# bencebecsy/pta_replicator

Hardware: AMD Instinct MI355X
Metric: realizations/sec, 68 psr x 5000 TOAs GWB+RN+WN (higher is better)
Workload: dtype f64; 1 GPU; BASELINE.json config 3: the 68 pulsars of ng15_dict.json x 5000 synthetic TOAs - HD GWB (gw_log10_A of the dict) + per-pulsar power-law RN (dict values, 30 components) + per-backend EFAC / t2EQUAD / ECORR (dict values), on-chip Philox draws, 1024 realisations per step per GPU; n_toa_total=340000, Nf=3000, npts=600, parallelism=replica-shard x1

## Files before the change

### pta_replicator_amd/csrc/pta_engine_kernels.hip

```cpp
#include "pta_common.h"
#include "pta_rng.h"
#include "pta_mfma.h"

__global__ void k_engine_rn_coef(uint64_t seed, uint64_t r0, int R, int P, int K, const double *__restrict__ amp,
                                 double *__restrict__ coef, int fast) {
  pta_rng_stage_tables();
  __syncthreads();
  int idx = blockIdx.x * blockDim.x + threadIdx.x;
  int hp = K / 2;
  int total = R * P * hp;
  if (idx >= total) return;
  int p = idx % hp, ra = idx / hp;
  int a = ra % P, r = ra / P;
  double z0, z1;
  pta_normal_pair(seed, r0 + (uint64_t)r, pta_stream_id(PTA_STREAM_RN, (uint32_t)a), (uint32_t)p, z0, z1, fast);
  int64_t o = (int64_t)ra * K + 2 * p;
  coef[o] = amp[(int64_t)a * K + 2 * p] * z0;
  coef[o + 1] = amp[(int64_t)a * K + 2 * p + 1] * z1;
}

extern "C" int pta_engine_rn_coef(uint64_t seed, uint64_t r0, int R, int P, int K, const double *amp, double *coef, int rng_fast,
                                  void *stream) {
  PTA_REQUIRE(amp && coef, PTA_E_ARG, "pta_engine_rn_coef: NULL argument");
  PTA_REQUIRE(R > 0 && P > 0 && K > 0 && (K % 2) == 0, PTA_E_ARG, "pta_engine_rn_coef: R=%d P=%d K=%d (K must be even)", R, P, K);
  int64_t total = (int64_t)R * P * (K / 2);
  PTA_REQUIRE(total < (1LL << 31), PTA_E_ARG, "pta_engine_rn_coef: problem too large");
  hipLaunchKernelGGL(k_engine_rn_coef, dim3(pta_cdiv(total, 256)), dim3(256), 0, pta_stream(stream), seed, r0, R, P, K, amp, coef, rng_fast ? 1 : 0);
  PTA_LAUNCH_CHECK();
  return PTA_OK;
}

#define ENG_RB 8

template <int MINW>
__global__ __launch_bounds__(PTA_ENGINE_TILE, MINW) void k_engine_synth(pta_engine_plan pl, uint64_t seed, uint64_t r0, int R,
                                                                  double *__restrict__ out, int64_t ld_out, int fast) {
  __shared__ double zec[ENG_RB][2 * PTA_ENGINE_EPMAX];
  pta_rng_stage_tables();
  __syncthreads();
  const int tile = blockIdx.y;
  const int rb = blockIdx.x * ENG_RB;
  const int a = pl.tile_psr[tile];
  const int start = pl.tile_start[tile];
  const int count = pl.tile_count[tile];
  const int t = threadIdx.x;
  const int P = pl.n_psr;
  const bool has_ec = pl.ecorr_toa != nullptr;
  const int epn = has_ec ? pl.tile_epn[tile] : 0;
  const int ep0 = has_ec ? pl.tile_ep0[tile] : 0;
  if (epn > 0) {
    const uint32_t strm = pta_stream_id(PTA_STREAM_ECORR, (uint32_t)a);
    for (int idx = t; idx < epn * ENG_RB; idx += PTA_ENGINE_TILE) {
      int q = idx / epn, p = idx - q * epn;
      double z0, z1;
      pta_normal_pair(seed, r0 + (uint64_t)(rb + q), strm, (uint32_t)(ep0 + p), z0, z1, fast);
      zec[q][2 * p] = z0;
      zec[q][2 * p + 1] = z1;
    }
    __syncthreads();
  }
  if (t >= count) return;
  const int i = start + t;
  double v[ENG_RB];
#pragma unroll
  for (int q = 0; q < ENG_RB; ++q) v[q] = 0.0;

  if (pl.rn_k > 0) {
    const int K = pl.rn_k;
    const double *__restrict__ Fcol = pl.Ft + i;
    const double *__restrict__ cf = pl.rn_coef + ((int64_t)rb * P + a) * K;
    const int64_t rstride = (int64_t)P * K;
    for (int c = 0; c < K; ++c) {
      double fv = Fcol[(int64_t)c * pl.ldf];
#pragma unroll
      for (int q = 0; q < ENG_RB; ++q) {
        int qq = (rb + q < R) ? q : 0;
        v[q] = fma(fv, cf[qq * rstride + c], v[q]);
      }
    }
  }
  if (pl.gw_npts > 0) {
    const int j = pl.gw_jlo[i];
    const double wgt = pl.gw_w[i];
    const double *__restrict__ gbase = pl.gw_G + ((int64_t)rb * P + a) * pl.gw_npts;
    const int64_t rstride = (int64_t)P * pl.gw_npts;
#pragma unroll
    for (int q = 0; q < ENG_RB; ++q) {
      int qq = (rb + q < R) ? q : 0;
      const double *g = gbase + qq * rstride;
      v[q] = v[q] + ((g[j + 1] - g[j]) * wgt + g[j]);
    }
  }
  if (pl.wn_a) {
    const double wa = pl.wn_a[i], wb = pl.wn_b[i];
    const uint32_t strm = pta_stream_id(PTA_STREAM_WN, (uint32_t)a);
    const uint32_t pair = (uint32_t)pl.idx_in_psr[i];
#pragma unroll
    for (int q = 0; q < ENG_RB; ++q) {
      double z1, z2;
      pta_normal_pair(seed, r0 + (uint64_t)(rb + q), strm, pair, z1, z2, fast);
      v[q] = v[q] + (wa * z1 + wb * z2);
    }
  }
  if (has_ec) {
    const double ec = pl.ecorr_toa[i];
    const int e = pl.epoch_of[i];
    if (epn > 0) {
      const int o = e - 2 * ep0;
#pragma unroll
      for (int q = 0; q < ENG_RB; ++q) v[q] = v[q] + ec * zec[q][o];
    } else if (ec != 0.0) {
      const uint32_t strm = pta_stream_id(PTA_STREAM_ECORR, (uint32_t)a);
#pragma unroll
      for (int q = 0; q < ENG_RB; ++q) v[q] = v[q] + ec * pta_normal_single(seed, r0 + (uint64_t)(rb + q), strm, (uint32_t)e, fast);
    }
  }
  const double det = pl.det ? pl.det[i] : 0.0;
#pragma unroll
  for (int q = 0; q < ENG_RB; ++q)
    if (rb + q < R) out[(int64_t)(rb + q) * ld_out + i] = v[q] + det;
}

typedef double pta_f64x2_a8 __attribute__((ext_vector_type(2), aligned(8)));
#define ENG_MR 16
#define ENG_ZPITCH (2 * PTA_ENGINE_EPMAX + 8)

struct pta_synth_ops {
  pta_f64x2_a8 y[4];
  double wgt, wa, wb, ec, det;
  uint32_t pair;
  int e, i;
};
template <bool FAST, bool SINGLE, bool RNIDX, int PF, int WPC, bool ALL>
__global__ __launch_bounds__(PTA_ENGINE_TILE, WPC) void k_engine_synth_mfma(pta_engine_plan pl, uint64_t seed, uint64_t r0, int R,
                                                                           double *__restrict__ out, int64_t ld_out, int xcd_aware) {
  constexpr int fast = FAST ? 1 : 0;
  __shared__ double zec[ENG_MR][ENG_ZPITCH];
  const int nrg = (R + ENG_MR - 1) / ENG_MR;
  const int64_t total = (int64_t)nrg * pl.n_tiles, chunk = (total + 7) >> 3;
  const int64_t item = xcd_aware ? (int64_t)(blockIdx.x & 7) * chunk + (blockIdx.x >> 3) : (int64_t)blockIdx.x;
  if (item >= total) return;
  pta_rng_stage_tables();
  __syncthreads();
  const int t = threadIdx.x, l = t & 63, wv = t >> 6;
  const int P = pl.n_psr;
  const bool has_ec = ALL || pl.ecorr_toa != nullptr;
  constexpr bool wn_single = SINGLE;
  const int col = l & 15, quad = l >> 4;
  const int tbase = wv * 64 + col;
  const int tile = (int)(item / nrg);
  const int rb = (int)(item - (int64_t)tile * nrg) * ENG_MR;
  const int a = pl.tile_psr[tile];
  const int start = pl.tile_start[tile];
  const int count = pl.tile_count[tile];
  const int epn = has_ec ? pl.tile_epn[tile] : 0;
  const int ep0 = has_ec ? pl.tile_ep0[tile] : 0;
  auto stage = [&]() {
    if (epn > 0) {
      const uint32_t strm = pta_stream_id(PTA_STREAM_ECORR, (uint32_t)a);
      for (int idx = t; idx < epn * ENG_MR; idx += PTA_ENGINE_TILE) {
        int q = idx / epn, p = idx - q * epn;
        double z0, z1;
        pta_normal_pair(seed, r0 + (uint64_t)(rb + q), strm, (uint32_t)(ep0 + p), z0, z1, fast);
        zec[q][2 * p] = z0;
        zec[q][2 * p + 1] = z1;
      }
      __syncthreads();
    }
  };
  if (PF == 0) stage();
  int rq[4];
#pragma unroll
  for (int g = 0; g < 4; ++g) rq[g] = min(quad + 4 * g, R - 1 - rb);
  int jl4[4];
#pragma unroll
  for (int j = 0; j < 4; ++j) jl4[j] = pl.gw_npts > 0 ? pl.gw_jlo[start + min(tbase + 16 * j, count - 1)] : 0;
  pta_f64x4 acc[4];
#pragma unroll
  for (int j = 0; j < 4; ++j) acc[j] = pta_f64x4{0.0, 0.0, 0.0, 0.0};
  const bool has_gw = ALL || pl.gw_npts > 0, has_wn = ALL || pl.wn_a != nullptr || wn_single;
  auto ldgw = [&](int j, pta_synth_ops &o) {
    const int i = start + min(tbase + 16 * j, count - 1);
    o.wgt = has_gw ? pl.gw_w[i] : 0.0;
    if (has_gw) {
#pragma unroll
      for (int g = 0; g < 4; ++g)
        o.y[g] = *reinterpret_cast<const pta_f64x2_a8 *>(pl.gw_G + ((int64_t)(rb + rq[g]) * P + a) * pl.gw_npts + jl4[j]);
    }
  };
  auto ldtoa = [&](int j, pta_synth_ops &o) {
    const int i = start + min(tbase + 16 * j, count - 1);
    o.i = i;
    o.wa = has_wn ? (wn_single ? pl.wn_c[i] : pl.wn_a[i]) : 0.0;
    o.wb = (has_wn && !wn_single) ? pl.wn_b[i] : 0.0;
    o.pair = (uint32_t)pl.idx_in_psr[i];
    o.ec = has_ec ? pl.ecorr_toa[i] : 0.0;
    o.e = has_ec ? pl.epoch_of[i] : 0;
    o.det = pl.det ? pl.det[i] : 0.0;
  };
  pta_synth_ops cur;
  auto mid = [&]() {
    if (PF & 4) ldgw(0, cur);
    if (PF & 1) ldtoa(0, cur);
    stage();
  };
  if (PF != 0 && !(PF & 2)) mid();
  if (pl.rn_k > 0) {
    const int K = pl.rn_k;
    const int ra = min(rb + col, R - 1);
    const double *__restrict__ cf = pl.rn_coef + ((int64_t)ra * P + a) * K;
    const double *__restrict__ Fb = pl.Ft + start;
    int tcl[4];
#pragma unroll
    for (int j = 0; j < 4; ++j) tcl[j] = min(tbase + 16 * j, count - 1);
    auto ld = [&](int k0, double &av, double (&bv)[4]) {
      const int k = k0 + quad, kc = min(k, K - 1);
      const double a_ld = cf[kc];
      av = (k < K) ? a_ld : 0.0;
      const double *__restrict__ Fk = Fb + (int64_t)kc * pl.ldf;
#pragma unroll
      for (int j = 0; j < 4; ++j) bv[j] = Fk[tcl[j]];
    };
    auto mm = [&](double av, const double (&bv)[4]) {
#pragma unroll
      for (int j = 0; j < 4; ++j) acc[j] = pta_mfma_f64(av, bv[j], acc[j]);
    };
    auto run = [&](auto &&ldx) {
      double a0, a1, a2, b0[4], b1[4], b2[4];
      ldx(0, a0, b0);
      ldx(4, a1, b1);
      if (PF & 2) mid();
      for (int k0 = 0; k0 < K; k0 += 12) {
        ldx(k0 + 8, a2, b2);
        mm(a0, b0);
        ldx(k0 + 12, a0, b0);
        mm(a1, b1);
        ldx(k0 + 16, a1, b1);
        mm(a2, b2);
      }
    };
    if (RNIDX) {
      const int klast = (K - 1) & ~3;
      const char *__restrict__ Fbytes = reinterpret_cast<const char *>(Fb);
      const char *__restrict__ cbytes = reinterpret_cast<const char *>(pl.rn_coef);
      const uint32_t ldfb = (uint32_t)pl.ldf * 8u;
      uint32_t offF[4];
#pragma unroll
      for (int j = 0; j < 4; ++j) offF[j] = (uint32_t)quad * ldfb + (uint32_t)tcl[j] * 8u;
      const uint32_t offC = (uint32_t)(((int64_t)ra * P + a) * K + quad) * 8u;
      const int kq = K - quad;
      auto ldu = [&](int k0, auto rowF, auto rowC, double &av, double (&bv)[4]) {
        const double a_ld = *reinterpret_cast<const double *>(cbytes + (uint32_t)(offC + rowC));
        av = (k0 < kq) ? a_ld : 0.0;
#pragma unroll
        for (int j = 0; j < 4; ++j) bv[j] = *reinterpret_cast<const double *>(Fbytes + (uint32_t)(offF[j] + rowF));
      };
      if ((K & 3) == 0) {
        run([&](int k0, double &av, double (&bv)[4]) {
          const uint32_t kg = (uint32_t)min(k0, klast);
          ldu(k0, kg * ldfb, kg * 8u, av, bv);
        });
      } else {
        const uint32_t dq = (uint32_t)(quad - min(quad, K - 1 - klast));
        run([&](int k0, double &av, double (&bv)[4]) {
          const uint32_t kg = (uint32_t)min(k0, klast);
          const uint32_t back = k0 >= klast ? dq : 0u;
          ldu(k0, kg * ldfb - back * ldfb, kg * 8u - back * 8u, av, bv);
        });
      }
    } else {
      run(ld);
    }
  } else if (PF & 2) {
    mid();
  }
  const uint32_t strm_wn = pta_stream_id(PTA_STREAM_WN, (uint32_t)a);
  const uint32_t strm_ec = pta_stream_id(PTA_STREAM_ECORR, (uint32_t)a);
  const bool wn_share = wn_single && count == PTA_ENGINE_TILE;
  double zs[4] = {0.0, 0.0, 0.0, 0.0};
  double pend[4] = {0.0, 0.0, 0.0, 0.0};
  int pend_i = 0;
#pragma unroll
  for (int j = 0; j < 4; ++j) {
    pta_synth_ops nxt;
    if (PF & 4) {
      if (!(PF & 1)) ldtoa(j, cur);
      if (j < 3) {
        ldgw(j + 1, nxt);
        if (PF & 1) ldtoa(j + 1, nxt);
      }
    }
    double wgt, wa, wb, ec, det;
    uint32_t pair;
    int e, i;
    pta_f64x2_a8 y[4];
    if (PF & 4) {
      wgt = cur.wgt, wa = cur.wa, wb = cur.wb, ec = cur.ec, det = cur.det, pair = cur.pair, e = cur.e, i = cur.i;
#pragma unroll
      for (int g = 0; g < 4; ++g) y[g] = cur.y[g];
    } else {
      i = start + min(tbase + 16 * j, count - 1);
      wgt = has_gw ? pl.gw_w[i] : 0.0;
      if (has_gw) {
#pragma unroll
        for (int g = 0; g < 4; ++g)
          y[g] = *reinterpret_cast<const pta_f64x2_a8 *>(pl.gw_G + ((int64_t)(rb + rq[g]) * P + a) * pl.gw_npts + jl4[j]);
      }
      wa = has_wn ? (wn_single ? pl.wn_c[i] : pl.wn_a[i]) : 0.0, wb = (has_wn && !wn_single) ? pl.wn_b[i] : 0.0;
      pair = (uint32_t)pl.idx_in_psr[i];
      ec = has_ec ? pl.ecorr_toa[i] : 0.0;
      e = has_ec ? pl.epoch_of[i] : 0;
      det = pl.det ? pl.det[i] : 0.0;
    }
    if (j > 0) {
#pragma unroll
      for (int g = 0; g < 4; ++g) out[(int64_t)(rb + rq[g]) * ld_out + pend_i] = pend[g];
    }
    double v[4];
#pragma unroll
    for (int g = 0; g < 4; ++g) v[g] = acc[j][g];
    if (has_gw) {
#pragma unroll
      for (int g = 0; g < 4; ++g) v[g] = v[g] + ((y[g].y - y[g].x) * wgt + y[g].x);
    }
    if (has_wn && !wn_single) {
#pragma unroll
      for (int g = 0; g < 4; ++g) {
        double z1, z2;
        pta_normal_pair(seed, r0 + (uint64_t)(rb + rq[g]), strm_wn, pair, z1, z2, fast);
        v[g] = v[g] + (wa * z1 + wb * z2);
      }
    } else if (wn_single) {
      const uint32_t pid = pair & ~16u;
      const bool br = (pair & 16u) != 0;
      const bool fresh = (j & 1) == 0 || !wn_share;
      if (fresh) {
#pragma unroll
        for (int g = 0; g < 4; ++g) {
          double z0, z1;
          pta_normal_pair(seed, r0 + (uint64_t)(rb + rq[g]), strm_wn, pid, z0, z1, fast);
          v[g] = v[g] + wa * (br ? z1 : z0);
          zs[g] = br ? z0 : z1;
        }
      } else {
#pragma unroll
        for (int g = 0; g < 4; ++g) v[g] = v[g] + wa * zs[g];
      }
    }
    if (has_ec) {
      if (epn > 0) {
        const int o = e - 2 * ep0;
#pragma unroll
        for (int g = 0; g < 4; ++g) v[g] = v[g] + ec * zec[rq[g]][o];
      }
#ifndef PTA_ISA_TABLE_MAIN_PATH_ONLY
      else if (ec != 0.0) {
#pragma unroll
        for (int g = 0; g < 4; ++g) v[g] = v[g] + ec * pta_normal_single(seed, r0 + (uint64_t)(rb + rq[g]), strm_ec, (uint32_t)e, fast);
      }
#endif
    }
#pragma unroll
    for (int g = 0; g < 4; ++g) pend[g] = v[g] + det;
    pend_i = i;
    if ((PF & 4) && j < 3) {
      cur.wgt = nxt.wgt;
#pragma unroll
      for (int g = 0; g < 4; ++g) cur.y[g] = nxt.y[g];
      if (PF & 1) cur = nxt;
    }
  }
#pragma unroll
  for (int g = 0; g < 4; ++g) out[(int64_t)(rb + rq[g]) * ld_out + pend_i] = pend[g];
}

typedef void (*pta_synth_fn)(pta_engine_plan, uint64_t, uint64_t, int, double *, int64_t, int);
template <bool FAST, bool SINGLE, bool RNIDX, int WPC, bool ALL>
static pta_synth_fn synth_kernel_pf(int pf) {
  if (pf == 0) return k_engine_synth_mfma<FAST, SINGLE, RNIDX, 0, WPC, ALL>;
  if (pf == 2) return k_engine_synth_mfma<FAST, SINGLE, RNIDX, 2, WPC, ALL>;
  if constexpr (WPC == 3) {
    if (pf == 4) return k_engine_synth_mfma<FAST, SINGLE, RNIDX, 4, WPC, ALL>;
    if (pf == 6) return k_engine_synth_mfma<FAST, SINGLE, RNIDX, 6, WPC, ALL>;
    if constexpr (!SINGLE) {
      if (pf == 5) return k_engine_synth_mfma<FAST, SINGLE, RNIDX, 5, WPC, ALL>;
      if (pf == 7) return k_engine_synth_mfma<FAST, SINGLE, RNIDX, 7, WPC, ALL>;
    }
  }
  return nullptr;
}
template <bool RNIDX, bool ALL>
static pta_synth_fn synth_kernel(int rng_fast, bool single, int pf, bool w3) {
  if (single) return rng_fast ? synth_kernel_pf<true, true, RNIDX, 3, ALL>(pf) : synth_kernel_pf<false, true, RNIDX, 3, ALL>(pf);
  if (w3) return rng_fast ? synth_kernel_pf<true, false, RNIDX, 3, ALL>(pf) : synth_kernel_pf<false, false, RNIDX, 3, ALL>(pf);
  return rng_fast ? synth_kernel_pf<true, false, RNIDX, 4, ALL>(pf) : synth_kernel_pf<false, false, RNIDX, 4, ALL>(pf);
}
#define PTA_SYNTH_DEFAULT_PF 0
#define PTA_SYNTH_DEFAULT_WPC 4

extern "C" int pta_engine_synth(const pta_engine_plan *plan_host, uint64_t seed, uint64_t r0, int R, double *out, int64_t ld_out,
                                void *stream) {
  PTA_REQUIRE(plan_host && out, PTA_E_ARG, "pta_engine_synth: NULL argument");
  const pta_engine_plan &p = *plan_host;
  PTA_REQUIRE(p.n_toa > 0 && p.n_psr > 0 && R > 0 && ld_out >= p.n_toa, PTA_E_ARG, "pta_engine_synth: n_toa=%d n_psr=%d R=%d", p.n_toa,
              p.n_psr, R);
  PTA_REQUIRE(p.n_tiles > 0 && p.tile_psr && p.tile_start && p.tile_count && p.tile_ep0 && p.tile_epn && p.idx_in_psr, PTA_E_ARG,
              "pta_engine_synth: tile table / idx_in_psr missing");
  PTA_REQUIRE(p.rn_k == 0 || (p.Ft && p.rn_coef && p.ldf >= p.n_toa), PTA_E_ARG, "pta_engine_synth: red-noise inputs missing");
  PTA_REQUIRE(p.gw_npts == 0 || (p.gw_G && p.gw_jlo && p.gw_w && p.gw_npts >= 2), PTA_E_ARG,
              "pta_engine_synth: GWB inputs missing");
  PTA_REQUIRE(!p.wn_a || p.wn_b, PTA_E_ARG, "pta_engine_synth: wn_b missing");
  PTA_REQUIRE(!p.wn_c || !p.wn_a, PTA_E_ARG, "pta_engine_synth: wn_c (single-deviate white noise) replaces wn_a / wn_b - pass one or the other");
  PTA_REQUIRE(!p.ecorr_toa || p.epoch_of, PTA_E_ARG, "pta_engine_synth: epoch_of missing");
  const int variant = p.synth_variant;
  const int rng_fast = p.rng_fast ? 1 : 0;
  const bool pipe = variant >= 16 && variant <= 79;
  PTA_REQUIRE(!pipe || (((variant - 16) & 7) != 1 && ((variant - 16) & 7) != 3), PTA_E_ARG,
              "pta_engine_synth: synth_variant %d - per-TOA operands ahead (bit 0) exist with the GWB operands ahead (bit 2) only", variant);
  if (variant == 0 || variant == 1 || variant == 2 || pipe || (variant >= 100 && variant <= 164)) {
    const int xcd = variant == 1 ? 0 : 1;
    const unsigned pad = variant >= 100 ? (unsigned)(variant - 100) * 1024u : 0u;
    const int64_t total = (int64_t)pta_cdiv(R, ENG_MR) * p.n_tiles, nwg = ((total + 7) >> 3) << 3;
    PTA_REQUIRE(nwg < (1LL << 31), PTA_E_ARG, "pta_engine_synth: %lld workgroups exceed one launch", (long long)nwg);
    const bool noidx = variant == 2 || (pipe && ((variant - 16) & 16));
    const bool rnidx = !noidx && p.rn_k > 0 && p.ldf < (1LL << 28) && ((int64_t)p.rn_k * p.ldf + PTA_ENGINE_TILE) * 8 < (1LL << 32) &&
                       (int64_t)R * p.n_psr * p.rn_k * 8 < (1LL << 32);
    const int pf = pipe ? (variant - 16) & 7 : variant == 2 ? 0 : PTA_SYNTH_DEFAULT_PF;
    const bool w3 = p.wn_c || (pipe ? ((variant - 16) & 8) != 0 : variant == 2 ? false : PTA_SYNTH_DEFAULT_WPC == 3);
    const bool all = !(pipe && ((variant - 16) & 32)) && variant != 2 && p.gw_npts > 0 && (p.wn_a || p.wn_c) && p.ecorr_toa;
    pta_synth_fn kern = all ? (rnidx ? synth_kernel<true, true>(rng_fast, p.wn_c != nullptr, pf, w3) : synth_kernel<false, true>(rng_fast, p.wn_c != nullptr, pf, w3))
                            : (rnidx ? synth_kernel<true, false>(rng_fast, p.wn_c != nullptr, pf, w3) : synth_kernel<false, false>(rng_fast, p.wn_c != nullptr, pf, w3));
    PTA_REQUIRE(kern, PTA_E_ARG, "pta_engine_synth: synth_variant %d - no kernel with pipelining %d at %d workgroups per CU%s (scratch)", variant, pf,
                w3 ? 3 : 4, p.wn_c ? ", single-deviate white noise" : "");
    hipLaunchKernelGGL(kern, dim3((unsigned)nwg), dim3(PTA_ENGINE_TILE), pad, pta_stream(stream), p, seed, r0, R, out, ld_out, xcd);
    PTA_LAUNCH_CHECK();
    return PTA_OK;
  }
  PTA_REQUIRE(!p.wn_c, PTA_E_ARG, "pta_engine_synth: the single-deviate white noise exists in the MFMA kernel only");
  PTA_REQUIRE(p.n_tiles <= 65535, PTA_E_ARG, "pta_engine_synth: %d tiles exceed the 2-D launch of the all-VALU kernel", p.n_tiles);
  dim3 g(pta_cdiv(R, ENG_RB), p.n_tiles), b(PTA_ENGINE_TILE);
  if (variant >= 8)
    hipLaunchKernelGGL(k_engine_synth<8>, g, b, 0, pta_stream(stream), p, seed, r0, R, out, ld_out, rng_fast);
  else if (variant >= 6)
    hipLaunchKernelGGL(k_engine_synth<6>, g, b, 0, pta_stream(stream), p, seed, r0, R, out, ld_out, rng_fast);
  else
    hipLaunchKernelGGL(k_engine_synth<4>, g, b, 0, pta_stream(stream), p, seed, r0, R, out, ld_out, rng_fast);
  PTA_LAUNCH_CHECK();
  return PTA_OK;
}

extern "C" int pta_gwb_czt(uint64_t seed, uint64_t r0, const double *w, int64_t ldw, int R, int P, int Nf, int npts, int i0,
                           const double *pre, const double *FB, const double *tw, const double *post, double *G0, int64_t ldg,
                           int variant, int rng_fast, void *stream);
extern "C" int pta_gwb_idft_rng(uint64_t seed, uint64_t r0, int R, int P, int Nf, const double *Tsym, const double *rot, int npts,
                                double *G0, int64_t ldg, int variant, int rng_fast, void *stream);
extern "C" int pta_gwb_mix(const double *Mchol, int P, const double *G0, int R, int npts, int64_t ldg, double *G, int variant,
                           void *stream);

static int engine_generate(const char *fn, const pta_engine_plan *plan_host, const pta_engine_tables *tables_host,
                           const pta_engine_hyper *hyper, uint64_t seed, uint64_t r0, int R, double *out, int64_t ld_out, void *stream) {
  PTA_REQUIRE(plan_host && tables_host && out, PTA_E_ARG, "%s: NULL argument", fn);
  const pta_engine_hyper fixed{};
  const pta_engine_hyper &h = hyper ? *hyper : fixed;
  pta_engine_plan p = *plan_host;
  const pta_engine_tables &tb = *tables_host;
  int rc;
  if (p.rn_k > 0) {
    PTA_REQUIRE(tb.rn_amp && tb.ws_coef, PTA_E_ARG, "%s: red-noise amplitudes / workspace missing", fn);
    if (h.rn_log10_A) {
      PTA_REQUIRE(h.rn_gamma && h.rn_f && h.rn_tspan, PTA_E_ARG, "%s: rn_gamma / rn_f / rn_tspan missing", fn);
      rc = pta_engine_rn_coef_hyper(seed, r0, R, p.n_psr, p.rn_k, h.rn_f, h.rn_tspan, h.rn_log10_A, h.rn_gamma, tb.rn_amp, tb.ws_coef,
                                    p.rng_fast, stream);
    } else {
      rc = pta_engine_rn_coef(seed, r0, R, p.n_psr, p.rn_k, tb.rn_amp, tb.ws_coef, p.rng_fast, stream);
    }
    if (rc != PTA_OK) return rc;
    p.rn_coef = tb.ws_coef;
  }
  if (p.gw_npts > 0) {
    PTA_REQUIRE(tb.Mchol && tb.ws_G0 && tb.ws_G, PTA_E_ARG, "%s: GWB factor / workspace missing", fn);
    const double *scale = h.gw_scale;
    if (!scale && h.gw_log10_A) {
      PTA_REQUIRE(h.gw_gamma && h.gw_f && h.gw_hcf0 && h.ws_scale, PTA_E_ARG, "%s: gw_gamma / gw_f / gw_hcf0 / ws_scale missing", fn);
      rc = pta_gwb_spectrum_scale(h.gw_f, h.gw_hcf0, tb.gw_nf, R, h.gw_log10_A, h.gw_gamma, h.gw_turnover, h.gw_f0, h.gw_beta,
                                  h.gw_power, h.ws_scale, h.ld_gw_scale, stream);
      if (rc != PTA_OK) return rc;
      scale = h.ws_scale;
    }
    if (tb.use_czt) {
      PTA_REQUIRE(tb.czt_pre && tb.czt_FB && tb.czt_tw && tb.czt_post, PTA_E_ARG, "%s: chirp-z tables missing", fn);
      rc = scale ? pta_gwb_czt_scaled(seed, r0, nullptr, 0, R, p.n_psr, tb.gw_nf, p.gw_npts, tb.gw_i0, tb.czt_pre, tb.czt_FB, tb.czt_tw,
                                      tb.czt_post, tb.ws_G0, p.gw_npts, tb.czt_variant, p.rng_fast, scale, h.ld_gw_scale, stream)
                 : pta_gwb_czt(seed, r0, nullptr, 0, R, p.n_psr, tb.gw_nf, p.gw_npts, tb.gw_i0, tb.czt_pre, tb.czt_FB, tb.czt_tw,
                               tb.czt_post, tb.ws_G0, p.gw_npts, tb.czt_variant, p.rng_fast, stream);
    } else {
      PTA_REQUIRE(tb.Tsym && tb.rot, PTA_E_ARG, "%s: DFT-GEMM tables missing", fn);
      rc = scale ? pta_gwb_idft_rng_scaled(seed, r0, R, p.n_psr, tb.gw_nf, tb.Tsym, tb.rot, p.gw_npts, tb.ws_G0, p.gw_npts, tb.idft_variant,
                                           p.rng_fast, scale, h.ld_gw_scale, stream)
                 : pta_gwb_idft_rng(seed, r0, R, p.n_psr, tb.gw_nf, tb.Tsym, tb.rot, p.gw_npts, tb.ws_G0, p.gw_npts, tb.idft_variant,
                                    p.rng_fast, stream);
    }
    if (rc != PTA_OK) return rc;
    rc = pta_gwb_mix(tb.Mchol, p.n_psr, tb.ws_G0, R, p.gw_npts, p.gw_npts, tb.ws_G, tb.mix_variant, stream);
    if (rc != PTA_OK) return rc;
    p.gw_G = tb.ws_G;
  }
  return pta_engine_synth(&p, seed, r0, R, out, ld_out, stream);
}

extern "C" int pta_engine_generate(const pta_engine_plan *plan_host, const pta_engine_tables *tables_host, uint64_t seed, uint64_t r0,
                                   int R, double *out, int64_t ld_out, void *stream) {
  return engine_generate("pta_engine_generate", plan_host, tables_host, nullptr, seed, r0, R, out, ld_out, stream);
}

extern "C" int pta_engine_generate_hyper(const pta_engine_plan *plan_host, const pta_engine_tables *tables_host,
                                         const pta_engine_hyper *hyper_host, uint64_t seed, uint64_t r0, int R, double *out,
                                         int64_t ld_out, void *stream) {
  PTA_REQUIRE(hyper_host, PTA_E_ARG, "pta_engine_generate_hyper: NULL argument");
  return engine_generate("pta_engine_generate_hyper", plan_host, tables_host, hyper_host, seed, r0, R, out, ld_out, stream);
}
```

### pta_replicator_amd/csrc/pta_rng.h

```cpp
#pragma once
#include <stdint.h>
#include <math.h>
#include "pta_rng_tables.h"

#ifndef PTA_HD
#if defined(__HIPCC__)
#define PTA_HD __host__ __device__ __forceinline__
#else
#define PTA_HD inline
#endif
#endif

#define PTA_STREAM_GWB 1u
#define PTA_STREAM_RN 2u
#define PTA_STREAM_WN 3u
#define PTA_STREAM_ECORR 4u
#define PTA_STREAM_TD 5u
#define PTA_STREAM_TDGW 6u
#define PTA_STREAM_HYPER 7u
#define PTA_STREAM_CW 8u

PTA_HD uint32_t pta_stream_id(uint32_t kind, uint32_t pulsar) { return (kind << 24) | (pulsar & 0xFFFFFFu); }

struct pta_u32x4 {
  uint32_t x, y, z, w;
};

PTA_HD void pta_mulhilo32(uint32_t a, uint32_t b, uint32_t &hi, uint32_t &lo) {
  uint64_t p = (uint64_t)a * (uint64_t)b;
  hi = (uint32_t)(p >> 32);
  lo = (uint32_t)p;
}

PTA_HD uint32_t pta_xor3(uint32_t a, uint32_t b, uint32_t c) {
#if defined(__HIP_DEVICE_COMPILE__)
  return __builtin_amdgcn_bitop3_b32(a, b, c, 0x96);
#else
  return a ^ b ^ c;
#endif
}

PTA_HD pta_u32x4 pta_philox4x32_10(pta_u32x4 c, uint32_t k0, uint32_t k1) {
#pragma unroll
  for (int r = 0; r < 10; ++r) {
    uint32_t hi0, lo0, hi1, lo1;
    pta_mulhilo32(0xD2511F53u, c.x, hi0, lo0);
    pta_mulhilo32(0xCD9E8D57u, c.z, hi1, lo1);
    pta_u32x4 n;
    n.x = pta_xor3(hi1, c.y, k0);
    n.y = lo1;
    n.z = pta_xor3(hi0, c.w, k1);
    n.w = lo0;
    c = n;
    k0 += 0x9E3779B9u;
    k1 += 0xBB67AE85u;
  }
  return c;
}

PTA_HD pta_u32x4 pta_philox_draw(uint64_t seed, uint64_t realisation, uint32_t stream, uint32_t pair) {
  pta_u32x4 c;
  c.x = pair;
  c.y = stream;
  c.z = (uint32_t)realisation;
  c.w = (uint32_t)(realisation >> 32);
  return pta_philox4x32_10(c, (uint32_t)seed, (uint32_t)(seed >> 32));
}

PTA_HD double pta_bits_to_double(uint64_t b) {
  double d;
  __builtin_memcpy(&d, &b, sizeof(d));
  return d;
}
PTA_HD uint64_t pta_double_to_bits(double d) {
  uint64_t b;
  __builtin_memcpy(&b, &d, sizeof(b));
  return b;
}

PTA_HD void pta_uniform_pair(pta_u32x4 v, double &u1, double &u2) {
  uint64_t a = ((((uint64_t)v.x << 32) | v.y) >> 12) | 0x3FF0000000000000ull;
  uint64_t b = ((((uint64_t)v.z << 32) | v.w) >> 12) | 0x3FF0000000000000ull;
  u1 = 2.0 - pta_bits_to_double(a);
  u2 = pta_bits_to_double(b) - 1.0;
}

PTA_HD double pta_fma_k(double x, double p, double c) {
#if defined(__HIP_DEVICE_COMPILE__)
  double d;
  asm("v_fma_f64 %0, %1, %2, %3" : "=v"(d) : "v"(x), "v"(p), "s"(c));
  return d;
#else
  return fma(x, p, c);
#endif
}

PTA_HD double pta_div(double x, double y) {
#if defined(__HIP_DEVICE_COMPILE__)
  double r = __builtin_amdgcn_rcp(y);
  r = fma(fma(-y, r, 1.0), r, r);
  double q = x * r;
  return fma(fma(-y, q, x), r, q);
#else
  return x / y;
#endif
}
PTA_HD double pta_sqrt_pos(double x) {
#if defined(__HIP_DEVICE_COMPILE__)
  x = fmax(x, 1e-300);
  double r = __builtin_amdgcn_rsq(x);
  double g = x * r, h = 0.5 * r;
  double d = fma(-h, g, 0.5);
  g = fma(g, d, g);
  h = fma(h, d, h);
  return fma(fma(-g, g, x), h, g);
#else
  return sqrt(fmax(x, 1e-300));
#endif
}

PTA_HD double pta_neg2log_poly(double u) {
  const double ln2_hi = 6.93147180369123816490e-01, ln2_lo = 1.90821492927058770002e-10;
  const double Lg1 = 6.666666666666735130e-01, Lg2 = 3.999999999940941908e-01, Lg3 = 2.857142874366239149e-01,
               Lg4 = 2.222219843214978396e-01, Lg5 = 1.818357216161805012e-01, Lg6 = 1.531383769920937332e-01,
               Lg7 = 1.479819860511658591e-01;
  uint64_t b = pta_double_to_bits(u);
  int e = (int)(b >> 52) - 1023;
  double m = pta_bits_to_double((b & 0x000FFFFFFFFFFFFFull) | 0x3FF0000000000000ull);
  if (m > 1.4142135623730951) {
    m *= 0.5;
    e += 1;
  }
  double f = m - 1.0;
  double s = pta_div(f, 2.0 + f);
  double z = s * s, w = z * z;
  double t1 = w * pta_fma_k(w, fma(w, Lg6, Lg4), Lg2);
  double t2 = z * pta_fma_k(w, pta_fma_k(w, fma(w, Lg7, Lg5), Lg3), Lg1);
  double R = t2 + t1;
  double hfsq = 0.5 * f * f;
  double dk = (double)e;
  double lnu = dk * ln2_hi - ((hfsq - fma(s, hfsq + R, dk * ln2_lo)) - f);
  return -2.0 * lnu;
}

PTA_HD void pta_sincos_2pi_poly(double u, double &sn, double &cs) {
  const double S1 = -1.66666666666666324348e-01, S2 = 8.33333333332248946124e-03, S3 = -1.98412698298579493134e-04,
               S4 = 2.75573137070700676789e-06, S5 = -2.50507602534068634195e-08, S6 = 1.58969099521155010221e-10;
  const double C1 = 4.16666666666666019037e-02, C2 = -1.38888888888741095749e-03, C3 = 2.48015872894767294178e-05,
               C4 = -2.75573143513906633035e-07, C5 = 2.08757232129817482790e-09, C6 = -1.13596475577881948265e-11;
  double q = rint(4.0 * u);
  double r = u - 0.25 * q;
  double x = 6.283185307179586 * r;
  double z = x * x;
  double ps = pta_fma_k(z, pta_fma_k(z, pta_fma_k(z, pta_fma_k(z, fma(z, S6, S5), S4), S3), S2), S1);
  double s = fma(x * z, ps, x);
  double pc = z * pta_fma_k(z, pta_fma_k(z, pta_fma_k(z, pta_fma_k(z, fma(z, C6, C5), C4), C3), C2), C1);
  double c = 1.0 - (0.5 * z - z * pc);
  int k = (int)q & 3;
  double s1 = (k & 1) ? c : s;
  double c1 = (k & 1) ? s : c;
  sn = (k == 2 || k == 3) ? -s1 : s1;
  cs = (k == 1 || k == 2) ? -c1 : c1;
}


#if defined(__HIP_DEVICE_COMPILE__)
__device__ __forceinline__ double *pta_rng_lds() {
  __shared__ double __attribute__((aligned(16))) tab[PTA_RNG_TAB_DOUBLES];
  return tab;
}
__device__ __forceinline__ void pta_rng_stage_tables() {
  double *t = pta_rng_lds();
  for (int i = threadIdx.x + blockDim.x * (threadIdx.y + blockDim.y * threadIdx.z); i < PTA_RNG_TAB_DOUBLES; i += blockDim.x * blockDim.y * blockDim.z)
    t[i] = pta_rng_tab[i];
}
#define PTA_RNG_TABLE pta_rng_lds()
#else
PTA_HD void pta_rng_stage_tables() {}
#define PTA_RNG_TABLE pta_rng_tab
#endif

PTA_HD double pta_neg2log(double u) {
  const double L2H = 1.38629436073824763298e+00, L2L = 3.81642985854117540004e-10;
  const uint64_t b = pta_double_to_bits(u);
  const uint32_t hi = (uint32_t)(b >> 32);
  const uint32_t j = (hi >> (20 - PTA_RNG_LOG_BITS)) & ((1u << PTA_RNG_LOG_BITS) - 1u);
  const int nk = 1023 - (int)((hi + (((1u << PTA_RNG_LOG_BITS) - PTA_RNG_LOG_CENTRED) << (20 - PTA_RNG_LOG_BITS))) >> 20);
  const uint32_t hi2 = hi + ((uint32_t)nk << 20);
  const double m = pta_bits_to_double(((uint64_t)hi2 << 32) | (b & 0xFFFFFFFFull));
  const double *e = PTA_RNG_TABLE + 2 * j;
  const double c = e[0], T = e[1];
  const double r = fma(m, c, -1.0);
  const double W = pta_fma_k(r, pta_fma_k(r, pta_fma_k(r, pta_fma_k(r, fma(r, -2.85714285714285698425e-01, 3.33333333333333314830e-01),
                                                   -4.00000000000000022204e-01), 0.5), -6.66666666666666629659e-01), 1.0);
  const double t = fma(r * r, W, -2.0 * r);
  const double nkd = (double)nk;
  return fma(nkd, L2H, T + fma(nkd, L2L, t));
}

PTA_HD void pta_sincos_2pi(double u, double &sn, double &cs) {
  const double kd = rint((double)PTA_RNG_SC_N * u);
  const double r = fma(kd, -1.0 / PTA_RNG_SC_N, u);
  const int k = (int)kd & (PTA_RNG_SC_N - 1);
  const double *e = PTA_RNG_TABLE + PTA_RNG_SC_OFF + 2 * k;
  const double sa = e[0], ca = e[1];
  const double x = 6.283185307179586 * r;
  const double z = x * x;
  const double ps = pta_fma_k(z, pta_fma_k(z, pta_fma_k(z, fma(z, 2.75573192239858925110e-06, -1.98412698412698412526e-04), 8.33333333333333321769e-03),
                                       -1.66666666666666657415e-01), 1.0);
  const double cx = pta_fma_k(z, pta_fma_k(z, pta_fma_k(z, fma(z, 2.48015873015873015658e-05, -1.38888888888888894189e-03), 4.16666666666666643537e-02),
                                       -0.5), 1.0);
  const double sx = x * ps;
  sn = fma(sa, cx, ca * sx);
  cs = fma(ca, cx, -(sa * sx));
}

PTA_HD void pta_normal_pair(uint64_t seed, uint64_t realisation, uint32_t stream, uint32_t pair, double &z0, double &z1, int fast = 0) {
  double u1, u2, s, c;
  pta_uniform_pair(pta_philox_draw(seed, realisation, stream, pair), u1, u2);
  if (fast) {
#if defined(__HIP_DEVICE_COMPILE__)
    float rad = __builtin_amdgcn_sqrtf(-1.3862943611198906f * __builtin_amdgcn_logf((float)u1));
    float x = (float)u2;
    z0 = (double)(rad * __builtin_amdgcn_cosf(x));
    z1 = (double)(rad * __builtin_amdgcn_sinf(x));
#else
    float rad = sqrtf(-1.3862943611198906f * log2f((float)u1));
    float x = 6.2831853071795864769f * (float)u2;
    z0 = (double)(rad * cosf(x));
    z1 = (double)(rad * sinf(x));
#endif
    return;
  }
  double rad = pta_sqrt_pos(pta_neg2log(u1));
  pta_sincos_2pi(u2, s, c);
  z0 = rad * c;
  z1 = rad * s;
}

PTA_HD double pta_normal_single(uint64_t seed, uint64_t realisation, uint32_t stream, uint32_t e, int fast = 0) {
  double z0, z1;
  pta_normal_pair(seed, realisation, stream, e >> 1, z0, z1, fast);
  return (e & 1u) ? z1 : z0;
}
```

Baseline: 216,400 realizations/s.

## Split first Philox round into per-realisation and per-pair halves shared via LDS

```diff
diff --git a/pta_replicator_amd/csrc/pta_engine_kernels.hip b/pta_replicator_amd/csrc/pta_engine_kernels.hip
--- a/pta_replicator_amd/csrc/pta_engine_kernels.hip
+++ b/pta_replicator_amd/csrc/pta_engine_kernels.hip
@@ -1,6 +1,7 @@
 #include "pta_common.h"
 #include "pta_rng.h"
 #include "pta_mfma.h"
+#include <type_traits>
 
 __global__ void k_engine_rn_coef(uint64_t seed, uint64_t r0, int R, int P, int K, const double *__restrict__ amp,
                                  double *__restrict__ coef, int fast) {
@@ -131,7 +132,11 @@
   uint32_t pair;
   int e, i;
 };
-template <bool FAST, bool SINGLE, bool RNIDX, int PF, int WPC, bool ALL>
+__device__ __forceinline__ uint4 *pta_synth_rhalf_lds() {
+  __shared__ uint4 tab[2 * ENG_MR];
+  return tab;
+}
+template <bool FAST, bool SINGLE, bool RNIDX, int PF, int WPC, bool ALL, bool SPLIT = false>
 __global__ __launch_bounds__(PTA_ENGINE_TILE, WPC) void k_engine_synth_mfma(pta_engine_plan pl, uint64_t seed, uint64_t r0, int R,
                                                                            double *__restrict__ out, int64_t ld_out, int xcd_aware) {
   constexpr int fast = FAST ? 1 : 0;
@@ -141,22 +146,47 @@
   const int64_t item = xcd_aware ? (int64_t)(blockIdx.x & 7) * chunk + (blockIdx.x >> 3) : (int64_t)blockIdx.x;
   if (item >= total) return;
   pta_rng_stage_tables();
+  const int t = threadIdx.x, l = t & 63, wv = t >> 6;
+  const int tile = (int)(item / nrg);
+  const int rb = (int)(item - (int64_t)tile * nrg) * ENG_MR;
+  const int a = pl.tile_psr[tile];
+  const uint32_t r_hi = (uint32_t)((r0 + (uint64_t)rb) >> 32);
+  const bool split_ok = SPLIT && r_hi == (uint32_t)((r0 + (uint64_t)rb + (ENG_MR - 1)) >> 32);
+  if constexpr (SPLIT) {
+    if (t < 2 * ENG_MR) {
+      const bool is_ec = t >= ENG_MR;
+      const int q = is_ec ? t - ENG_MR : min(t, R - 1 - rb);
+      const pta_philox_half B = pta_philox_real_half((uint32_t)(r0 + (uint64_t)(rb + q)), pta_stream_id(is_ec ? PTA_STREAM_ECORR : PTA_STREAM_WN, (uint32_t)a), seed);
+      pta_synth_rhalf_lds()[t] = make_uint4(B.a, B.b, B.c, 0u);
+    }
+  }
   __syncthreads();
-  const int t = threadIdx.x, l = t & 63, wv = t >> 6;
+  auto body = [&](auto sp_c) {
+  constexpr bool SP = decltype(sp_c)::value;
   const int P = pl.n_psr;
   const bool has_ec = ALL || pl.ecorr_toa != nullptr;
   constexpr bool wn_single = SINGLE;
   const int col = l & 15, quad = l >> 4;
   const int tbase = wv * 64 + col;
-  const int tile = (int)(item / nrg);
-  const int rb = (int)(item - (int64_t)tile * nrg) * ENG_MR;
-  const int a = pl.tile_psr[tile];
   const int start = pl.tile_start[tile];
   const int count = pl.tile_count[tile];
   const int epn = has_ec ? pl.tile_epn[tile] : 0;
   const int ep0 = has_ec ? pl.tile_ep0[tile] : 0;
   auto stage = [&]() {
     if (epn > 0) {
+      if constexpr (SP) {
+        const int q = t >> 4;
+        const uint4 b = pta_synth_rhalf_lds()[ENG_MR + q];
+        const pta_philox_half B = {b.x, b.y, b.z};
+        for (int p = t & 15; p < epn; p += 16) {
+          double z0, z1;
+          pta_normal_pair_split(pta_philox_pair_half((uint32_t)(ep0 + p), r_hi, seed), B, seed, z0, z1, fast);
+          zec[q][2 * p] = z0;
+          zec[q][2 * p + 1] = z1;
+        }
+        __syncthreads();
+        return;
+      }
       const uint32_t strm = pta_stream_id(PTA_STREAM_ECORR, (uint32_t)a);
       for (int idx = t; idx < epn * ENG_MR; idx += PTA_ENGINE_TILE) {
         int q = idx / epn, p = idx - q * epn;
@@ -280,6 +310,11 @@
   double zs[4] = {0.0, 0.0, 0.0, 0.0};
   double pend[4] = {0.0, 0.0, 0.0, 0.0};
   int pend_i = 0;
+  [[maybe_unused]] const uint4 *rhalf = pta_synth_rhalf_lds() + quad;
+  auto draw = [&](pta_philox_half A, int g, double &z0, double &z1) {
+    const uint4 b = rhalf[4 * g];
+    pta_normal_pair_split(A, pta_philox_half{b.x, b.y, b.z}, seed, z0, z1, fast);
+  };
 #pragma unroll
   for (int j = 0; j < 4; ++j) {
     pta_synth_ops nxt;
@@ -324,10 +359,13 @@
       for (int g = 0; g < 4; ++g) v[g] = v[g] + ((y[g].y - y[g].x) * wgt + y[g].x);
     }
     if (has_wn && !wn_single) {
+      pta_philox_half A;
+      if constexpr (SP) A = pta_philox_pair_half(pair, r_hi, seed);
 #pragma unroll
       for (int g = 0; g < 4; ++g) {
         double z1, z2;
-        pta_normal_pair(seed, r0 + (uint64_t)(rb + rq[g]), strm_wn, pair, z1, z2, fast);
+        if constexpr (SP) draw(A, g, z1, z2);
+        else pta_normal_pair(seed, r0 + (uint64_t)(rb + rq[g]), strm_wn, pair, z1, z2, fast);
         v[g] = v[g] + (wa * z1 + wb * z2);
       }
     } else if (wn_single) {
@@ -335,10 +373,13 @@
       const bool br = (pair & 16u) != 0;
       const bool fresh = (j & 1) == 0 || !wn_share;
       if (fresh) {
+        pta_philox_half A;
+        if constexpr (SP) A = pta_philox_pair_half(pid, r_hi, seed);
 #pragma unroll
         for (int g = 0; g < 4; ++g) {
           double z0, z1;
-          pta_normal_pair(seed, r0 + (uint64_t)(rb + rq[g]), strm_wn, pid, z0, z1, fast);
+          if constexpr (SP) draw(A, g, z0, z1);
+          else pta_normal_pair(seed, r0 + (uint64_t)(rb + rq[g]), strm_wn, pid, z0, z1, fast);
           v[g] = v[g] + wa * (br ? z1 : z0);
           zs[g] = br ? z0 : z1;
         }
@@ -372,11 +413,23 @@
   }
 #pragma unroll
   for (int g = 0; g < 4; ++g) out[(int64_t)(rb + rq[g]) * ld_out + pend_i] = pend[g];
+  };
+  if constexpr (SPLIT) {
+    if (split_ok) body(std::true_type{});
+    else body(std::false_type{});
+  } else {
+    body(std::false_type{});
+  }
 }
 
 typedef void (*pta_synth_fn)(pta_engine_plan, uint64_t, uint64_t, int, double *, int64_t, int);
 template <bool FAST, bool SINGLE, bool RNIDX, int WPC, bool ALL>
-static pta_synth_fn synth_kernel_pf(int pf) {
+static pta_synth_fn synth_kernel_pf(int pf, bool split) {
+  if constexpr (WPC == 4 || SINGLE) {
+    if (split) return pf == 0 ? k_engine_synth_mfma<FAST, SINGLE, RNIDX, 0, WPC, ALL, true> : nullptr;
+  } else {
+    if (split) return nullptr;
+  }
   if (pf == 0) return k_engine_synth_mfma<FAST, SINGLE, RNIDX, 0, WPC, ALL>;
   if (pf == 2) return k_engine_synth_mfma<FAST, SINGLE, RNIDX, 2, WPC, ALL>;
   if constexpr (WPC == 3) {
@@ -390,10 +443,10 @@
   return nullptr;
 }
 template <bool RNIDX, bool ALL>
-static pta_synth_fn synth_kernel(int rng_fast, bool single, int pf, bool w3) {
-  if (single) return rng_fast ? synth_kernel_pf<true, true, RNIDX, 3, ALL>(pf) : synth_kernel_pf<false, true, RNIDX, 3, ALL>(pf);
-  if (w3) return rng_fast ? synth_kernel_pf<true, false, RNIDX, 3, ALL>(pf) : synth_kernel_pf<false, false, RNIDX, 3, ALL>(pf);
-  return rng_fast ? synth_kernel_pf<true, false, RNIDX, 4, ALL>(pf) : synth_kernel_pf<false, false, RNIDX, 4, ALL>(pf);
+static pta_synth_fn synth_kernel(int rng_fast, bool single, int pf, bool w3, bool split) {
+  if (single) return rng_fast ? synth_kernel_pf<true, true, RNIDX, 3, ALL>(pf, split) : synth_kernel_pf<false, true, RNIDX, 3, ALL>(pf, split);
+  if (w3) return rng_fast ? synth_kernel_pf<true, false, RNIDX, 3, ALL>(pf, split) : synth_kernel_pf<false, false, RNIDX, 3, ALL>(pf, split);
+  return rng_fast ? synth_kernel_pf<true, false, RNIDX, 4, ALL>(pf, split) : synth_kernel_pf<false, false, RNIDX, 4, ALL>(pf, split);
 }
 #define PTA_SYNTH_DEFAULT_PF 0
 #define PTA_SYNTH_DEFAULT_WPC 4
@@ -417,7 +470,7 @@
   const bool pipe = variant >= 16 && variant <= 79;
   PTA_REQUIRE(!pipe || (((variant - 16) & 7) != 1 && ((variant - 16) & 7) != 3), PTA_E_ARG,
               "pta_engine_synth: synth_variant %d - per-TOA operands ahead (bit 0) exist with the GWB operands ahead (bit 2) only", variant);
-  if (variant == 0 || variant == 1 || variant == 2 || pipe || (variant >= 100 && variant <= 164)) {
+  if (variant == 0 || variant == 1 || variant == 2 || variant == 3 || pipe || (variant >= 100 && variant <= 164)) {
     const int xcd = variant == 1 ? 0 : 1;
     const unsigned pad = variant >= 100 ? (unsigned)(variant - 100) * 1024u : 0u;
     const int64_t total = (int64_t)pta_cdiv(R, ENG_MR) * p.n_tiles, nwg = ((total + 7) >> 3) << 3;
@@ -427,9 +480,10 @@
                        (int64_t)R * p.n_psr * p.rn_k * 8 < (1LL << 32);
     const int pf = pipe ? (variant - 16) & 7 : variant == 2 ? 0 : PTA_SYNTH_DEFAULT_PF;
     const bool w3 = p.wn_c || (pipe ? ((variant - 16) & 8) != 0 : variant == 2 ? false : PTA_SYNTH_DEFAULT_WPC == 3);
+    const bool split = variant == 0 || variant == 1 || variant >= 100;
     const bool all = !(pipe && ((variant - 16) & 32)) && variant != 2 && p.gw_npts > 0 && (p.wn_a || p.wn_c) && p.ecorr_toa;
-    pta_synth_fn kern = all ? (rnidx ? synth_kernel<true, true>(rng_fast, p.wn_c != nullptr, pf, w3) : synth_kernel<false, true>(rng_fast, p.wn_c != nullptr, pf, w3))
-                            : (rnidx ? synth_kernel<true, false>(rng_fast, p.wn_c != nullptr, pf, w3) : synth_kernel<false, false>(rng_fast, p.wn_c != nullptr, pf, w3));
+    pta_synth_fn kern = all ? (rnidx ? synth_kernel<true, true>(rng_fast, p.wn_c != nullptr, pf, w3, split) : synth_kernel<false, true>(rng_fast, p.wn_c != nullptr, pf, w3, split))
+                            : (rnidx ? synth_kernel<true, false>(rng_fast, p.wn_c != nullptr, pf, w3, split) : synth_kernel<false, false>(rng_fast, p.wn_c != nullptr, pf, w3, split));
     PTA_REQUIRE(kern, PTA_E_ARG, "pta_engine_synth: synth_variant %d - no kernel with pipelining %d at %d workgroups per CU%s (scratch)", variant, pf,
                 w3 ? 3 : 4, p.wn_c ? ", single-deviate white noise" : "");
     hipLaunchKernelGGL(kern, dim3((unsigned)nwg), dim3(PTA_ENGINE_TILE), pad, pta_stream(stream), p, seed, r0, R, out, ld_out, xcd);
diff --git a/pta_replicator_amd/csrc/pta_rng.h b/pta_replicator_amd/csrc/pta_rng.h
--- a/pta_replicator_amd/csrc/pta_rng.h
+++ b/pta_replicator_amd/csrc/pta_rng.h
@@ -67,6 +67,48 @@
   return pta_philox4x32_10(c, (uint32_t)seed, (uint32_t)(seed >> 32));
 }
 
+struct pta_philox_half {
+  uint32_t a, b, c;
+};
+PTA_HD pta_philox_half pta_philox_pair_half(uint32_t pair, uint32_t realisation_hi, uint64_t seed) {
+  uint32_t hi0, lo0;
+  pta_philox_half h;
+  pta_mulhilo32(0xD2511F53u, pair, hi0, lo0);
+  pta_mulhilo32(0xCD9E8D57u, pta_xor3(hi0, realisation_hi, (uint32_t)(seed >> 32)), h.a, h.b);
+  h.c = lo0;
+  return h;
+}
+PTA_HD pta_philox_half pta_philox_real_half(uint32_t realisation_lo, uint32_t stream, uint64_t seed) {
+  uint32_t hi1;
+  pta_philox_half h;
+  pta_mulhilo32(0xCD9E8D57u, realisation_lo, hi1, h.a);
+  pta_mulhilo32(0xD2511F53u, pta_xor3(hi1, stream, (uint32_t)seed), h.b, h.c);
+  return h;
+}
+PTA_HD pta_u32x4 pta_philox_join(pta_philox_half A, pta_philox_half B, uint64_t seed) {
+  uint32_t k0 = (uint32_t)seed + 0x9E3779B9u, k1 = (uint32_t)(seed >> 32) + 0xBB67AE85u;
+  pta_u32x4 c;
+  c.x = pta_xor3(A.a, B.a, k0);
+  c.y = A.b;
+  c.z = pta_xor3(B.b, A.c, k1);
+  c.w = B.c;
+#pragma unroll
+  for (int r = 2; r < 10; ++r) {
+    k0 += 0x9E3779B9u;
+    k1 += 0xBB67AE85u;
+    uint32_t hi0, lo0, hi1, lo1;
+    pta_mulhilo32(0xD2511F53u, c.x, hi0, lo0);
+    pta_mulhilo32(0xCD9E8D57u, c.z, hi1, lo1);
+    pta_u32x4 n;
+    n.x = pta_xor3(hi1, c.y, k0);
+    n.y = lo1;
+    n.z = pta_xor3(hi0, c.w, k1);
+    n.w = lo0;
+    c = n;
+  }
+  return c;
+}
+
 PTA_HD double pta_bits_to_double(uint64_t b) {
   double d;
   __builtin_memcpy(&d, &b, sizeof(d));
@@ -78,9 +120,16 @@
   return b;
 }
 
+PTA_HD uint64_t pta_mantissa_12(uint32_t x, uint32_t y) {
+#if defined(__HIP_DEVICE_COMPILE__)
+  return ((uint64_t)__builtin_amdgcn_alignbit(0x3FFu, x, 12) << 32) | __builtin_amdgcn_alignbit(x, y, 12);
+#else
+  return ((((uint64_t)x << 32) | y) >> 12) | 0x3FF0000000000000ull;
+#endif
+}
 PTA_HD void pta_uniform_pair(pta_u32x4 v, double &u1, double &u2) {
-  uint64_t a = ((((uint64_t)v.x << 32) | v.y) >> 12) | 0x3FF0000000000000ull;
-  uint64_t b = ((((uint64_t)v.z << 32) | v.w) >> 12) | 0x3FF0000000000000ull;
+  uint64_t a = pta_mantissa_12(v.x, v.y);
+  uint64_t b = pta_mantissa_12(v.z, v.w);
   u1 = 2.0 - pta_bits_to_double(a);
   u2 = pta_bits_to_double(b) - 1.0;
 }
@@ -215,9 +264,9 @@
   cs = fma(ca, cx, -(sa * sx));
 }
 
-PTA_HD void pta_normal_pair(uint64_t seed, uint64_t realisation, uint32_t stream, uint32_t pair, double &z0, double &z1, int fast = 0) {
+PTA_HD void pta_box_muller(pta_u32x4 bits, double &z0, double &z1, int fast) {
   double u1, u2, s, c;
-  pta_uniform_pair(pta_philox_draw(seed, realisation, stream, pair), u1, u2);
+  pta_uniform_pair(bits, u1, u2);
   if (fast) {
 #if defined(__HIP_DEVICE_COMPILE__)
     float rad = __builtin_amdgcn_sqrtf(-1.3862943611198906f * __builtin_amdgcn_logf((float)u1));
@@ -237,6 +286,12 @@
   z0 = rad * c;
   z1 = rad * s;
 }
+PTA_HD void pta_normal_pair(uint64_t seed, uint64_t realisation, uint32_t stream, uint32_t pair, double &z0, double &z1, int fast = 0) {
+  pta_box_muller(pta_philox_draw(seed, realisation, stream, pair), z0, z1, fast);
+}
+PTA_HD void pta_normal_pair_split(pta_philox_half A, pta_philox_half B, uint64_t seed, double &z0, double &z1, int fast = 0) {
+  pta_box_muller(pta_philox_join(A, B, seed), z0, z1, fast);
+}
 
 PTA_HD double pta_normal_single(uint64_t seed, uint64_t realisation, uint32_t stream, uint32_t e, int fast = 0) {
   double z0, z1;
```

Measured after the change: 217,600 realizations/s (median of 6 runs). Within noise of the previous version (+0.6%).
